# johannes-graeter/limo

Hardware: NVIDIA H100
Metric: BA windows/s (30 KF, 3k LM, 40k obs) (higher is better)
Workload: dtype f64

## Files before the change

limo_b200/csrc/kba_device.cuh:

```cuda
#pragma once
#include <cstdint>
#include <cuda_runtime.h>

namespace kba {

constexpr int kMaxKf = 128;
constexpr int kMaxCam = 8;
constexpr int kPoseStride = 12;
constexpr int kCamStride = 16;
constexpr int kIterLogCap = 160;
constexpr int kFusedMaxKf = 32;

struct WinDesc {
    int n_kf, n_cam, n_lm, n_obs, n_gp;
    int kf_off, cam_off, lm_off, obs_off, gp_off;
    int chunk_off, n_chunks;
    int grp_off, n_groups;
    int scale_kf0, scale_kf1;
    double scale_weight, scale_value;
    double plane_reg_weight;
    int plane_dist_fixed, landmarks_fixed;
    int speed_kf, pad0;
    double speed_weight, speed_dt;
    double speed_v_before[3];
// ... 320 lines not shown
#pragma unroll
    for (int i = 0; i < 3; ++i) {
        T m0, m1, m2;
        if (i == 0) { m0 = fz * (cam[0] - xn * cam[6]); m1 = fz * (cam[1] - xn * cam[7]); m2 = fz * (cam[2] - xn * cam[8]); }
        else if (i == 1) { m0 = fz * (cam[3] - yn * cam[6]); m1 = fz * (cam[4] - yn * cam[7]); m2 = fz * (cam[5] - yn * cam[8]); }
        else { m0 = sqd * cam[6]; m1 = sqd * cam[7]; m2 = sqd * cam[8]; }
        if (write_jp) {
            T* o = jp + (size_t)(6 * i) * stride;
            lin_store<T, kCs>(o, T(-2) * (m1 * a2 - m2 * a1));
            lin_store<T, kCs>(o + stride, T(-2) * (m2 * a0 - m0 * a2));
            lin_store<T, kCs>(o + 2 * stride, T(-2) * (m0 * a1 - m1 * a0));
            lin_store<T, kCs>(o + 3 * stride, m0);
            lin_store<T, kCs>(o + 4 * stride, m1);
            lin_store<T, kCs>(o + 5 * stride, m2);
        }
        if (kJl) {
            T* q = jl + (size_t)(3 * i) * stride;
            lin_store<T, kCs>(q, m0 * pose[0] + m1 * pose[3] + m2 * pose[6]);
            lin_store<T, kCs>(q + stride, m0 * pose[1] + m1 * pose[4] + m2 * pose[7]);
            lin_store<T, kCs>(q + 2 * stride, m0 * pose[2] + m1 * pose[5] + m2 * pose[8]);
        }
    }
    return true;
}

__device__ __forceinline__ double lin_load(const double* base, size_t idx, int precision) {
    return precision ? (double)reinterpret_cast<const float*>(base)[idx] : base[idx];
}

__device__ inline void stage_window(const WinDesc& wd, const double* __restrict__ pose7, const double* __restrict__ cam16,
                                    double* s_pose, double* s_cam) {
    for (int k = threadIdx.x; k < wd.n_kf; k += blockDim.x) {
        const double* p = pose7 + 7 * (size_t)(wd.kf_off + k);
        double R[9];
        quat_to_rot<double>(p, R);
#pragma unroll
        for (int i = 0; i < 9; ++i) s_pose[kPoseStride * k + i] = R[i];
        s_pose[kPoseStride * k + 9] = p[4];
        s_pose[kPoseStride * k + 10] = p[5];
        s_pose[kPoseStride * k + 11] = p[6];
    }
    for (int i = threadIdx.x; i < wd.n_cam * kCamStride; i += blockDim.x) s_cam[i] = cam16[(size_t)wd.cam_off * kCamStride + i];
}

__device__ inline void write_rt(double* rt12, const double* p7) {
    quat_to_rot<double>(p7, rt12);
    rt12[9] = p7[4]; rt12[10] = p7[5]; rt12[11] = p7[6];
}

__device__ __forceinline__ size_t vobs_index(size_t obs_off, int p0, int p1, int o, int c) {
    return 18 * (obs_off + (size_t)p0) + (size_t)(6 * (p1 - p0)) * c + (size_t)6 * (o - p0);
}

__device__ __forceinline__ uint32_t smem_u32(const void* p) { return (uint32_t)__cvta_generic_to_shared(p); }
__device__ __forceinline__ void mbar_init(uint64_t* bar, int count) {
    asm volatile("mbarrier.init.shared::cta.b64 [%0], %1;" ::"r"(smem_u32(bar)), "r"(count));
}
__device__ __forceinline__ void mbar_expect_tx(uint64_t* bar, uint32_t bytes) {
    asm volatile("mbarrier.arrive.expect_tx.shared::cta.b64 _, [%0], %1;" ::"r"(smem_u32(bar)), "r"(bytes) : "memory");
}
__device__ __forceinline__ void tma_load_1d(void* dst, const void* src, uint32_t bytes, uint64_t* bar) {
    asm volatile("cp.async.bulk.shared::cluster.global.mbarrier::complete_tx::bytes [%0], [%1], %2, [%3];" ::"r"(smem_u32(dst)),
                 "l"(src), "r"(bytes), "r"(smem_u32(bar))
                 : "memory");
}
__device__ __forceinline__ void mbar_wait(uint64_t* bar, uint32_t parity) {
    uint32_t done = 0;
    while (!done)
        asm volatile("{\n.reg .pred p;\nmbarrier.try_wait.parity.shared::cta.b64 p, [%1], %2;\nselp.u32 %0, 1, 0, p;\n}"
                     : "=r"(done)
                     : "r"(smem_u32(bar)), "r"(parity)
                     : "memory");
}

__device__ inline void stage_window_bulk(const WinDesc& wd, const double* __restrict__ rt, const double* __restrict__ cam16,
                                         double* s_pose, double* s_cam, uint64_t* bar) {
    if (threadIdx.x == 0) {
        mbar_init(bar, 1);
        asm volatile("fence.proxy.async.shared::cta;" ::: "memory");
    }
    __syncthreads();
    if (threadIdx.x == 0) {
        const uint32_t bp = (uint32_t)(wd.n_kf * kPoseStride * sizeof(double)), bc = (uint32_t)(wd.n_cam * kCamStride * sizeof(double));
        mbar_expect_tx(bar, bp + bc);
        tma_load_1d(s_pose, rt + (size_t)kPoseStride * wd.kf_off, bp, bar);
        tma_load_1d(s_cam, cam16 + (size_t)kCamStride * wd.cam_off, bc, bar);
    }
    mbar_wait(bar, 0);
}

__device__ inline double warp_sum(double v) {
#pragma unroll
    for (int o = 16; o > 0; o >>= 1) v += __shfl_xor_sync(0xffffffffu, v, o);
    return v;
}
__device__ inline double warp_max(double v) {
#pragma unroll
    for (int o = 16; o > 0; o >>= 1) v = fmax(v, __shfl_xor_sync(0xffffffffu, v, o));
    return v;
}

}
```

limo_b200/csrc/kba_kernels.cu:

```cuda
#include "kba_device.cuh"
#include "kba_kernels.h"
#include "kba_regularisers.cuh"
#include "kba_prep.cuh"
#include "kba_linearize.cuh"

#include <cfloat>
#include <cstdio>
#include <cstdlib>
#include <cmath>
#include <type_traits>

namespace kba {

constexpr int kBeginThreads = 1024;
__global__ void __launch_bounds__(kBeginThreads) k_solve_begin(BatchDev bd, SolveParams sp) {
    const int w = blockIdx.x;
    WinState& st = bd.state[w];
    if (st.phase != PH_SOLVE_BEGIN) return;
    const WinDesc wd = bd.desc[w];
    __shared__ int s_has[kMaxKf];
    __shared__ int s_plane[kMaxKf];
    __shared__ int s_cnt[3];
    __shared__ int s_tile_chunk[513];
    for (int k = threadIdx.x; k < wd.n_kf; k += blockDim.x) { s_has[k] = 0; s_plane[k] = 0; }
// ... 1478 lines not shown
            if (off < 0) continue;
            if (bd.obs_rank[base + o] != 0) continue;
            const double* q = pcol + (off - prow0);
#pragma unroll
            for (int r = 0; r < 6; ++r) {
                const double d = delta_f[off + r];
                t[0] += q[r] * d; t[1] += q[prs + r] * d; t[2] += q[2 * prs + r] * d;
            }
        }
    }
    const unsigned any = __ballot_sync(0xffffffffu, mine) & (0xffffu << (threadIdx.x & 16));
    if (gl >= 0 && hl < 10 && !(any != 0u && hl < 6)) {
        const int row = gp_row(bd, wd, bd.gp_kf[wd.gp_off + gl], hl);
        if (row >= 0) {
            const double d = delta_f[row];
#pragma unroll
            for (int c = 0; c < 3; ++c) t[c] += bd.vgp[(size_t)(3 * hl + c) * bd.tot_gp + wd.gp_off + gl] * d;
        }
    }
#pragma unroll
    for (int c = 0; c < 3; ++c)
#pragma unroll
        for (int m = 8; m >= 1; m >>= 1) t[c] += __shfl_xor_sync(0xffffffffu, t[c], m);
    if (have && hl == 0) {
        if (!in) {
            pn[0] = pc[0]; pn[1] = pc[1]; pn[2] = pc[2];
        } else {
            const double* z = bd.lm_z + 3 * (size_t)L;
            const double* li = bd.lm_linv + 6 * (size_t)L;
            const double t0 = t[0] + z[0], t1 = t[1] + z[1], t2 = t[2] + z[2];
            const double d0 = -(li[0] * t0 + li[1] * t1 + li[3] * t2);
            const double d1 = -(li[2] * t1 + li[4] * t2);
            const double d2 = -(li[5] * t2);
            const double* g = bd.lm_g + 3 * (size_t)L;
            const double* lam = bd.lm_lambda + 3 * (size_t)L;
            pn[0] = pc[0] + d0; pn[1] = pc[1] + d1; pn[2] = pc[2] + d2;
            model = -(g[0] * d0 + g[1] * d1 + g[2] * d2) + lam[0] * d0 * d0 + lam[1] * d1 * d1 + lam[2] * d2 * d2;
            step_sq = d0 * d0 + d1 * d1 + d2 * d2;
            xn_sq = pc[0] * pc[0] + pc[1] * pc[1] + pc[2] * pc[2];
            gmax = fmax(fabs(g[0]), fmax(fabs(g[1]), fabs(g[2])));
            if (!isfinite(d0) || !isfinite(d1) || !isfinite(d2)) model = nan("");
        }
    }
    if (hl == 0) { s_red[grp][0] = model; s_red[grp][1] = step_sq; s_red[grp][2] = xn_sq; s_red[grp][3] = gmax; }
    __syncthreads();
    if (threadIdx.x == 0) {
        double a = 0, b = 0, c = 0, g = 0;
        for (int q = 0; q < 16; ++q) { a += s_red[q][0]; b += s_red[q][1]; c += s_red[q][2]; g = fmax(g, s_red[q][3]); }
        double* out = bd.bs_part + ((size_t)w * bd.bs_parts + blockIdx.x) * 4;
        out[0] = a; out[1] = b; out[2] = c; out[3] = g;
    }
}

template <bool kLoop>
__global__ void __launch_bounds__(256) k_backsub_v(BatchDev bd, int n_units) {
    const int w = blockIdx.y;
    const WinState& st = bd.state[w];
    if (st.phase != PH_ITERATE) return;
    const WinDesc& wd = bd.desc[w];
    __shared__ double s_red[16][4];
    const int hl = threadIdx.x & 15, grp = threadIdx.x >> 4;
    for (int unit = blockIdx.x; unit < n_units; unit += gridDim.x) {
    const int j = unit * 16 + grp;
    double model = 0.0, step_sq = 0.0, xn_sq = 0.0, gmax = 0.0;
    const bool have = j < wd.n_lm;
    const int L = wd.lm_off + (have ? j : 0);
    const double* pc = bd.lm[st.cur] + 3 * (size_t)L;
    double* pn = bd.lm[1 - st.cur] + 3 * (size_t)L;
    const int* lm_ptr = bd.lm_ptr + wd.lm_off + w;
    const int o0 = have ? lm_ptr[j] : 0, o1 = have ? lm_ptr[j + 1] : 0;
    const bool in = have && bd.lm_active[L] && o1 > o0 && !wd.landmarks_fixed && !st.solve_failed;
    const size_t base = (size_t)wd.obs_off;
    const double* delta_f = bd.delta_f + (size_t)w * bd.nr_cap_max;
    double t[3] = {0, 0, 0};
    if (in) {
        for (int o = o0 + hl; o < o1; o += 16) {
            const int off = bd.obs_row[base + o];
            if (off < 0) continue;
            double d[6];
#pragma unroll
            for (int r = 0; r < 6; ++r) d[r] = delta_f[off + r];
#pragma unroll
            for (int c = 0; c < 3; ++c) {
                const double2* v = reinterpret_cast<const double2*>(bd.vobs + vobs_index(base, o0, o1, o, c));
#pragma unroll
                for (int h = 0; h < 3; ++h) {
                    const double2 x = v[h];
                    t[c] += x.x * d[2 * h] + x.y * d[2 * h + 1];
                }
            }
        }
        const int gl = (wd.n_gp > 0) ? bd.gp_of_lm[L] : -1;
        if (gl >= 0 && hl < 10) {
            const int row = gp_row(bd, wd, bd.gp_kf[wd.gp_off + gl], hl);
            if (row >= 0) {
                const double d = delta_f[row];
#pragma unroll
                for (int c = 0; c < 3; ++c) t[c] += bd.vgp[(size_t)(3 * hl + c) * bd.tot_gp + wd.gp_off + gl] * d;
            }
        }
    }
#pragma unroll
    for (int c = 0; c < 3; ++c)
#pragma unroll
        for (int m = 8; m >= 1; m >>= 1) t[c] += __shfl_xor_sync(0xffffffffu, t[c], m);
    if (have && hl == 0) {
        if (!in) {
            pn[0] = pc[0]; pn[1] = pc[1]; pn[2] = pc[2];
        } else {
            const double* z = bd.lm_z + 3 * (size_t)L;
            const double* li = bd.lm_linv + 6 * (size_t)L;
            const double t0 = t[0] + z[0], t1 = t[1] + z[1], t2 = t[2] + z[2];
            const double d0 = -(li[0] * t0 + li[1] * t1 + li[3] * t2);
            const double d1 = -(li[2] * t1 + li[4] * t2);
            const double d2 = -(li[5] * t2);
            const double* g = bd.lm_g + 3 * (size_t)L;
            const double* lam = bd.lm_lambda + 3 * (size_t)L;
            pn[0] = pc[0] + d0; pn[1] = pc[1] + d1; pn[2] = pc[2] + d2;
            model = -(g[0] * d0 + g[1] * d1 + g[2] * d2) + lam[0] * d0 * d0 + lam[1] * d1 * d1 + lam[2] * d2 * d2;
            step_sq = d0 * d0 + d1 * d1 + d2 * d2;
            xn_sq = pc[0] * pc[0] + pc[1] * pc[1] + pc[2] * pc[2];
            gmax = fmax(fabs(g[0]), fmax(fabs(g[1]), fabs(g[2])));
            if (!isfinite(d0) || !isfinite(d1) || !isfinite(d2)) model = nan("");
        }
    }
    if (hl == 0) { s_red[grp][0] = model; s_red[grp][1] = step_sq; s_red[grp][2] = xn_sq; s_red[grp][3] = gmax; }
    __syncthreads();
    if (threadIdx.x == 0) {
        double a = 0, b = 0, c = 0, g = 0;
        for (int q = 0; q < 16; ++q) { a += s_red[q][0]; b += s_red[q][1]; c += s_red[q][2]; g = fmax(g, s_red[q][3]); }
        double* out = bd.bs_part + ((size_t)w * bd.bs_parts + unit) * 4;
        out[0] = a; out[1] = b; out[2] = c; out[3] = g;
    }
    if constexpr (!kLoop) break;
    if (unit + (int)gridDim.x < n_units) __syncthreads();
    }
}

__device__ void log_iter(BatchDev& bd, int w, WinState& st, double cost, double cost_change, double gmax,
                         double step_norm, double rel, double radius, int valid, int successful) {
    if (st.log_n >= kIterLogCap) return;
// ... 513 lines not shown
            k_landmark_reduce<true><<<dim3((bd.max_lm + 15) / 16, B), 256, 0, s>>>(bd, sp); LCHK("k_landmark_reduce");
            k_obs_v2<<<g_obs, 256, 0, s>>>(bd); LCHK("k_obs_v2");
        }
        const dim3 gf(bd.p_split, B);
        if (lc.fused_slots == 7) k_schur_fused<7><<<gf, 512, schur_fused_smem(), s>>>(bd);
        else k_schur_fused<6><<<gf, 512, schur_fused_smem(), s>>>(bd);
        LCHK("k_schur_fused");
    } else {
        k_landmark_reduce<false><<<dim3((bd.max_lm + 15) / 16, B), 256, 0, s>>>(bd, sp); LCHK("k_landmark_reduce");
        for (int round = 0; round <= lc.max_rank; ++round) k_obs_v<<<g_obs, 256, 0, s>>>(bd, round);
        LCHK("k_obs_v");
        if (bd.tot_gp > 0) k_gp_panel<<<dim3((bd.max_gp * 10 + 255) / 256, B), 256, 0, s>>>(bd);
        LCHK("k_gp_panel");
    }
    if (bd.fused) {
    } else if (lc.small_syrk) {
        k_schur_syrk_tma<<<dim3(bd.p_split, B), 512, schur_tma_smem(), s>>>(bd); LCHK("k_schur_syrk_tma");
    } else {
        const int nb = lc.nr_cap_max / 64;
        k_schur_syrk<<<dim3(nb * (nb + 1) / 2, bd.p_split, B), 256, schur_smem(), s>>>(bd); LCHK("k_schur_syrk");
    }
    const dim3 g_red((lc.nr_cap_max * lc.nr_cap_max + 255) / 256, B);
    BatchDev bc = bd;
    if (bd.sharded) {
        if (bd.p_split > 1) k_sred_reduce<<<g_red, 256, 0, s>>>(bd, 1);
        LCHK("k_sred_reduce");
        const LaunchCfg::WinDescHost& wh = lc.shard_win;
        const long long n_s = (long long)wh.nr_cap * wh.nr_cap, n_b = (long long)wh.n_kf * 27, n_x = n_s + n_b + bd.cost_parts + 2;
        k_shard_pack<<<(unsigned)((n_x + 255) / 256), 256, 0, s>>>(bd); LCHK("k_shard_pack");
        if (int rc = lc.xchg.allreduce(lc.xchg.user, bd.x_send, bd.x_recv, n_x, 0, s)) return rc;
        k_shard_flags<<<1, 32, 0, s>>>(bd); LCHK("k_shard_flags");
        bc.sred = bd.x_recv; bc.bkf = bd.x_recv + n_s; bc.cost_part_x = bd.x_recv + n_s + n_b;
        k_sred_reduce<<<g_red, 256, 0, s>>>(bc, 2); LCHK("k_sred_reduce");
    } else if (bd.p_split > 1) {
        k_sred_reduce<<<g_red, 256, 0, s>>>(bd, 0); LCHK("k_sred_reduce");
    }
    if (bd.solve_tiled) {
        k_reduced_solve<true><<<B, 512, solve_tiled_smem(lc.nr_cap_max), s>>>(bc, sp, 0); LCHK("k_reduced_solve");
    } else if (!bd.solve_split) {
        k_reduced_solve<false><<<B, 512, solve_smem(lc.nr_cap_max), s>>>(bc, sp, 0); LCHK("k_reduced_solve");
    } else {
        k_reduced_solve<false><<<B, 512, solve_smem(lc.nr_cap_max), s>>>(bc, sp, 1); LCHK("k_reduced_solve");
        const int strips = (lc.nr_cap_max + 7) / 8;
        for (int kb = 0; kb < lc.nr_cap_max; kb += kNB) {
            k_chol_diag<<<B, 32, 0, s>>>(bc, kb); LCHK("k_chol_diag");
            k_chol_panel<<<dim3((strips + 15) / 16, B), 512, 0, s>>>(bc, kb); LCHK("k_chol_panel");
            k_chol_trail<<<dim3(bd.solve_split, B), 512, trail_smem(lc.nr_cap_max), s>>>(bc, kb); LCHK("k_chol_trail");
        }
        k_reduced_solve<false><<<B, 512, solve_smem(lc.nr_cap_max), s>>>(bc, sp, 2); LCHK("k_reduced_solve");
    }
    if (bd.fused) {
        const int n_units = (bd.max_lm + 15) / 16;
        const int gx = strided_grid(lc.bs_grid, n_units, 1, 3, B, lc.sm_count, 2, 8);
        if (gx < n_units) k_backsub_v<true><<<dim3(gx, B), 256, 0, s>>>(bd, n_units);
        else k_backsub_v<false><<<dim3(n_units, B), 256, 0, s>>>(bd, n_units);
    }
    else k_backsub<<<dim3((bd.max_lm + 15) / 16, B), 256, 0, s>>>(bd);
    LCHK("k_backsub");
    launch_eval_obs<false>(bd, sp, s);
    if (bd.tot_gp > 0) k_gp_eval<false><<<B, 256, 0, s>>>(bd, sp);
    LCHK("k_gp_eval");
    if (bd.sharded) {
        k_shard_scalars<<<1, 256, 0, s>>>(bd); LCHK("k_shard_scalars");
        if (int rc = lc.xchg.allreduce(lc.xchg.user, bd.xs, bd.xs, 16 + bd.shard_world, 0, s)) return rc;
    }
    k_lm_update<<<(B * 32 + 127) / 128, 128, 0, s>>>(bd, sp); LCHK("k_lm_update");
    k_trim_eval<<<g_lm, 256, 0, s>>>(bd, sp); LCHK("k_trim_eval");
    if (bd.sharded) {
        k_shard_trim_scatter<<<(bd.max_lm + 255) / 256, 256, 0, s>>>(bd); LCHK("k_shard_trim_scatter");
        if (int rc = lc.xchg.allreduce(lc.xchg.user, bd.trim_send, bd.trim_glob, 3LL * bd.lm_total, 0, s)) return rc;
    }
    k_trim_select<<<B, 512, 0, s>>>(bd, sp); LCHK("k_trim_select");
    if (cnt) {
        const int gp = bd.tot_gp > 0 ? 1 : 0;
        const int prep = lin1 ? 1 : 2 + (bd.fused ? 1 : lc.max_rank + 1 + gp);
        const int split = (!bd.solve_tiled && bd.solve_split) ? 1 + 3 * ((lc.nr_cap_max + kNB - 1) / kNB) : 0;
        cnt->launches_total += (bd.fused ? 0 : 1) + 1 + 1 + gp + prep + 1 + (bd.p_split > 1 ? 1 : 0) + 1 + split + 1 + 1 + gp + 1 + 2;
        cnt->launches_jacobian += 1; cnt->launches_prep += prep + gp; cnt->launches_schur += 1; cnt->launches_solve += 2;
        cnt->launches_backsub += 1; cnt->launches_cost += 1 + gp; cnt->launches_update += 1; cnt->launches_trim += 2;
    }
    return 0;
}

void launch_count_active(const BatchDev& bd, cudaStream_t s) {
    cudaMemsetAsync(bd.n_active, 0, sizeof(int), s);
    k_count_active<<<(bd.n_win + 127) / 128, 128, 0, s>>>(bd); LCHK("k_count_active");
}

__global__ void __launch_bounds__(256) k_loop_cond(BatchDev bd, cudaGraphConditionalHandle handle, int* pass, int max_passes) {
    int active = 0;
    for (int w = threadIdx.x; w < bd.n_win; w += blockDim.x) active += (bd.state[w].phase != PH_DONE) ? 1 : 0;
    active = __syncthreads_count(active > 0);
    if (threadIdx.x == 0) {
        const int p = *pass + 1;
        *pass = p;
        *bd.n_active = active;
        cudaGraphSetConditional(handle, (active > 0 && p < max_passes) ? 1u : 0u);
    }
}
void launch_loop_cond(const BatchDev& bd, unsigned long long handle, int* pass, int max_passes, cudaStream_t s) {
    k_loop_cond<<<1, 256, 0, s>>>(bd, (cudaGraphConditionalHandle)handle, pass, max_passes);
}

__global__ void k_force_linearize(BatchDev bd) {
    const int w = blockIdx.x * blockDim.x + threadIdx.x;
    if (w >= bd.n_win) return;
    WinState& st = bd.state[w];
    st.phase = PH_ITERATE; st.need_linearize = 1; st.iter0 = 1; st.cur = 0; st.eval_failed = 0; st.solve_failed = 0;
// ... 31 lines not shown
```

limo_b200/csrc/kba_linearize.cuh:

```cuda
#pragma once
#include <type_traits>
#include "kba_device.cuh"

namespace kba {

constexpr int kLinThreads = 256;
constexpr int kLinWarps = kLinThreads / 32;

__host__ __device__ __forceinline__ int lin_tile_bound(int n_obs, int n_lm) { return n_obs / 16 + n_lm / 32 + 4; }
__device__ __forceinline__ size_t lin_tile_offset(const WinDesc& wd, int w) {
    return (size_t)(wd.obs_off / 16) + (size_t)(wd.lm_off / 32) + 4 * (size_t)w;
}

__device__ inline void build_lin_tiles(const BatchDev& bd, const WinDesc& wd, WinState& st, int w, int* s_chunk ) {
    const int* lm_ptr = bd.lm_ptr + wd.lm_off + w;
    int2* tiles = bd.lin_tile + lin_tile_offset(wd, w);
    const int per = max(64, (wd.n_lm + 511) / 512);
    const int n_chunks = (wd.n_lm + per - 1) / per;
    for (int pass = 0; pass < 2; ++pass) {
        for (int c = threadIdx.x; c < n_chunks; c += blockDim.x) {
            const int j0 = c * per, j1 = min(wd.n_lm, j0 + per);
            int n = 0, t_start = 0, t_cnt = 0;
            int2* out = tiles + (pass ? s_chunk[c] : 0);
            int o0 = lm_ptr[j0];
// ... 173 lines not shown
#pragma unroll
            for (int e = 0; e < 3; ++e) {
                tt[e] = st.iter0 ? 1.0 + sqrt(cd[e]) : tt_ld[e];
                const double t2 = tt[e] * tt[e];
                lam[e] = fmin(fmax(cd[e], sp.min_lm_diagonal * t2), sp.max_lm_diagonal * t2) * inv_radius;
            }
            const double a00 = c[0] + lam[0], a11 = c[3] + lam[1], a22 = c[5] + lam[2];
            const double i00 = rsqrt(a00);
            const double l10 = c[1] * i00, l20 = c[2] * i00;
            const double d11 = a11 - l10 * l10;
            const double i11 = rsqrt(d11);
            const double l21 = (c[4] - l20 * l10) * i11;
            const double d22 = a22 - l20 * l20 - l21 * l21;
            const double i22 = rsqrt(d22);
            if (!((a00 > 0.0) && (d11 > 0.0) && (d22 > 0.0))) {
                st.solve_failed = 1;
            } else {
                const double i10 = -l10 * i00 * i11;
                const double i21 = -l21 * i11 * i22;
                const double i20 = -(l20 * i00 + l21 * i10) * i22;
                if (first) {
                    double* li = bd.lm_linv + 6 * (size_t)L;
                    li[0] = i00; li[1] = i10; li[2] = i11; li[3] = i20; li[4] = i21; li[5] = i22;
                    double* zz = bd.lm_z + 3 * (size_t)L;
                    zz[0] = i00 * g[0]; zz[1] = i10 * g[0] + i11 * g[1]; zz[2] = i20 * g[0] + i21 * g[1] + i22 * g[2];
#pragma unroll
                    for (int e = 0; e < 3; ++e) {
                        bd.lm_g[3 * (size_t)L + e] = g[e];
                        bd.lm_lambda[3 * (size_t)L + e] = lam[e];
                        if (st.iter0) bd.lm_scale[3 * (size_t)L + e] = tt[e];
                    }
                    if (gl >= 0) {
                        for (int rr = 0; rr < 10; ++rr) {
                            const double jf_ = bd.gp_lin[(1 + rr) * TG + G];
                            const double e0 = jf_ * gjl[0], e1 = jf_ * gjl[1], e2 = jf_ * gjl[2];
                            bd.vgp[(3 * rr + 0) * TG + G] = e0 * i00;
                            bd.vgp[(3 * rr + 1) * TG + G] = e0 * i10 + e1 * i11;
                            bd.vgp[(3 * rr + 2) * TG + G] = e0 * i20 + e1 * i21 + e2 * i22;
                        }
                    }
                }
                if ((six[5][lane] & 128) && six[1][lane] >= 0) {
                    const double* R = s_pose + kPoseStride * six[0][lane];
                    const int g0 = six[2][lane];
                    double wm[9];
#pragma unroll
                    for (int r = 0; r < 3; ++r) {
                        const double m0 = sma[sym3(r, 0)], m1 = sma[sym3(r, 1)], m2 = sma[sym3(r, 2)];
                        const double l0 = m0 * R[0] + m1 * R[3] + m2 * R[6], l1 = m0 * R[1] + m1 * R[4] + m2 * R[7], l2 = m0 * R[2] + m1 * R[5] + m2 * R[8];
                        wm[3 * r + 0] = l0 * i00;
                        wm[3 * r + 1] = l0 * i10 + l1 * i11;
                        wm[3 * r + 2] = l0 * i20 + l1 * i21 + l2 * i22;
                    }
#pragma unroll
                    for (int cc = 0; cc < 3; ++cc) {
                        double2* out = reinterpret_cast<double2*>(bd.vobs + vobs_index(0, g0, g0 + klen, g0 + lane - seg0, cc));
                        const double w0 = wm[cc], w1 = wm[3 + cc], w2 = wm[6 + cc];
                        const double a0 = sma[6], a1 = sma[7], a2 = sma[8];
                        out[0] = make_double2(2.0 * (a1 * w2 - a2 * w1), 2.0 * (a2 * w0 - a0 * w2));
                        out[1] = make_double2(2.0 * (a0 * w1 - a1 * w0), w0);
                        out[2] = make_double2(w1, w2);
                    }
                }
            }
        }
    }
    __syncthreads();
    if (tid == 0) {
        double s = 0.0;
        int cnt = 0;
        for (int q = 0; q < kLinWarps; ++q) { s += s_red[q]; cnt += s_cnt[q]; }
        if (want_cost()) bd.cost_part_x[(size_t)w * bd.cost_parts + unit] = s;
        if (cnt) atomicAdd(bd.jac_obs, (unsigned long long)cnt);
    }
    if constexpr (!kLoop) break;
    if (unit + (int)gridDim.x < n_units) __syncthreads();
    }
}

}
```

limo_b200/csrc/kba_schur_fused.cuh:

```cuda
#pragma once

namespace kba {

constexpr int kLG = 8;
constexpr int kGC = 3 * kLG;
constexpr int kFStages = 6;
constexpr int kFMaxRs = 196;
constexpr int kFStageDoubles = kGC * kFMaxRs;
constexpr int kFObs = 128;
constexpr int kFConsumerWarps = 12;
constexpr int kFMaxKf = 32;

__constant__ signed char kSyrkMap12[12][7] = {
    {72, 7, 22, 33, 36, 48, 65}, {67, 10, 12, 19, 40, 53, -1}, {73, 1, 13, 17, 42, 50, -1}, {77, 8, 21, 26, 39, 54, -1},
    {75, 3, 18, 34, 49, 57, -1}, {69, 6, 23, 41, 58, 62, -1},  {66, 11, 27, 32, 38, 64, -1}, {74, 9, 20, 30, 37, 52, 55},
    {68, 0, 14, 16, 31, 44, 51}, {76, 2, 24, 29, 43, 45, 60},  {71, 5, 25, 28, 46, 56, 63},  {70, 4, 15, 35, 47, 59, 61}};

__device__ __forceinline__ void mbar_arrive(uint64_t* bar) {
    asm volatile("mbarrier.arrive.shared::cta.b64 _, [%0];" ::"r"(smem_u32(bar)) : "memory");
}
__device__ __forceinline__ void cp_async_elem(double* dst, const double* src) {
    asm volatile("cp.async.ca.shared.global [%0], [%1], 8;" ::"r"(smem_u32(dst)), "l"(src) : "memory");
}
__device__ __forceinline__ void cp_async_elem(float* dst, const float* src) {
    asm volatile("cp.async.ca.shared.global [%0], [%1], 4;" ::"r"(smem_u32(dst)), "l"(src) : "memory");
}
__device__ __forceinline__ void cp_async16(double* dst, const double* src) {
    asm volatile("cp.async.cg.shared.global [%0], [%1], 16;" ::"r"(smem_u32(dst)), "l"(src) : "memory");
}
__device__ __forceinline__ void cp_async8(double* dst, const double* src) {
    asm volatile("cp.async.ca.shared.global [%0], [%1], 8;" ::"r"(smem_u32(dst)), "l"(src) : "memory");
}
__device__ __forceinline__ void cp_async_arrive(uint64_t* bar) {
    asm volatile("cp.async.mbarrier.arrive.noinc.shared::cta.b64 [%0];" ::"r"(smem_u32(bar)) : "memory");
}
__device__ __forceinline__ void cp_async_commit() { asm volatile("cp.async.commit_group;" ::: "memory"); }
template <int N>
__device__ __forceinline__ void cp_async_wait() { asm volatile("cp.async.wait_group %0;" ::"n"(N) : "memory"); }
__device__ __forceinline__ void producer_sync() { asm volatile("bar.sync 1, 128;" ::: "memory"); }
template <int N>
__device__ __forceinline__ void reg_dec() { asm volatile("setmaxnreg.dec.sync.aligned.u32 %0;" ::"n"(N)); }
template <int N>
__device__ __forceinline__ void reg_inc() { asm volatile("setmaxnreg.inc.sync.aligned.u32 %0;" ::"n"(N)); }

constexpr size_t schur_fused_smem() { return (size_t)kFStages * kFStageDoubles * sizeof(double) + 24 * sizeof(uint64_t); }

#ifdef KBA_PROF
#define KBA_PROF_DECL long long pt_ = clock64(), pacc_[3] = {0, 0, 0}
#define KBA_PROF_T0 pt_ = clock64()
#define KBA_PROF_ACC(i) do { const long long n_ = clock64(); pacc_[i] += n_ - pt_; pt_ = n_; } while (0)
#define KBA_PROF_FLUSH(base) do { if (lane == 0 && bd.prof) for (int i_ = 0; i_ < 3; ++i_) atomicAdd(bd.prof + (base) + i_, (unsigned long long)pacc_[i_]); } while (0)
#else
#define KBA_PROF_DECL
#define KBA_PROF_T0
#define KBA_PROF_ACC(i)
#define KBA_PROF_FLUSH(base)
#endif

__device__ __forceinline__ void schur_split(int n_groups, int p_split, int& per, int& used) {
    per = max(8, (n_groups + p_split - 1) / p_split);
    used = max(1, min(p_split, (n_groups + per - 1) / per));
}

template <int kSlots>
__global__ void __launch_bounds__(512, 1) k_schur_fused(BatchDev bd) {
    const int w = blockIdx.y;
    const WinState& st = bd.state[w];
    if (st.phase != PH_ITERATE || st.solve_failed) return;
    const WinDesc& wd = bd.desc[w];
    if (wd.landmarks_fixed) return;
    extern __shared__ __align__(128) unsigned char fsm[];
    double* stage = reinterpret_cast<double*>(fsm);
    uint64_t* full = reinterpret_cast<uint64_t*>(fsm + (size_t)kFStages * kFStageDoubles * sizeof(double));
    uint64_t* empty = full + kFStages;
    const int tid = threadIdx.x, warp = tid >> 5, lane = tid & 31;
    const int n_f = st.n_f, nt = (n_f + 8) >> 3, trhs = n_f >> 3;
    int per, used;
    schur_split(wd.n_groups, (int)gridDim.x, per, used);
    if ((int)blockIdx.x >= used) return;
    const int g0 = blockIdx.x * per, g1 = min(wd.n_groups, g0 + per);
    const int* grs = bd.grp_rs + wd.grp_off;
    const int* gt0 = bd.grp_t0 + wd.grp_off;
    const int* gt1 = bd.grp_t1 + wd.grp_off;
    if (tid == 0) {
        for (int i = 0; i < kFStages; ++i) { mbar_init(&full[i], 1); mbar_init(&empty[i], kFConsumerWarps); }
        asm volatile("fence.proxy.async.shared::cta;" ::: "memory");
    }
    __syncthreads();
    auto next_group = [&](int g) { while (g < g1 && grs[g] == 0) ++g; return g; };

    if (warp >= kFConsumerWarps) {
        if (kSlots == 7) reg_dec<56>(); else reg_dec<104>();

        const int pw = warp - kFConsumerWarps;
        const int* lm_ptr = bd.lm_ptr + wd.lm_off + w;
        const size_t base = (size_t)wd.obs_off, TG = (size_t)bd.tot_gp;
        const bool sync_path = wd.n_gp > 0 || wd.max_rank > 0;
        const int cj = lane / 3, cc = lane - 3 * cj;
        const int zj = lane - 24;
        int g1_ = -1, rs1 = 0, t01 = 0, t11 = 0, act1 = 0, p01 = 0, p11 = 0;
        int4 run1 = make_int4(0, 0, 0, 0);
        KBA_PROF_DECL;
        auto load_meta = [&](int g) {
            g1_ = g; act1 = 0; run1 = make_int4(0, 0, 0, 0); p01 = p11 = 0;
            if (g >= g1) return;
            rs1 = grs[g]; t01 = gt0[g]; t11 = gt1[g];
            if (lane < 24) {
                const int j = g * kLG + cj;
                if (j < wd.n_lm) { run1 = bd.lm_run[wd.lm_off + j]; p01 = lm_ptr[j]; p11 = lm_ptr[j + 1]; }
            } else {
                const int j = g * kLG + zj;
                if (j < wd.n_lm) { act1 = bd.lm_active[wd.lm_off + j]; p01 = lm_ptr[j]; p11 = lm_ptr[j + 1]; }
            }
        };
        auto nth_group = [&](int g, int n) {
            g = next_group(g);
            for (; n > 0 && g < g1; --n) g = next_group(g + 1);
            return g;
        };
        int g = nth_group(g0, pw), gi = pw;
        load_meta(g);
        while (g < g1) {
            const int rs = rs1, t0 = t01, t1 = t11, act0 = act1, p00 = p01, p10 = p11;
            const int4 run0 = run1;
            const int gnext = nth_group(g + 1, 3);
            load_meta(gnext);
            const int slot = gi % kFStages;
            KBA_PROF_T0;
            if (gi >= kFStages) mbar_wait(&empty[slot], ((gi / kFStages) - 1) & 1);
            KBA_PROF_ACC(0);
            double* sb = stage + (size_t)slot * kFStageDoubles;
            {
                const int h = rs >> 1;
                for (int c = 0; c < kGC; ++c)
                    for (int r2 = lane; r2 < h; r2 += 32) reinterpret_cast<double2*>(sb + (size_t)c * kFMaxRs)[r2] = make_double2(0.0, 0.0);
            }
            const bool no_run = lane < 24 && (run0.y < 0 || (run0.y > 0 && ((run0.z - 8 * t0) & 1)));
            const bool bulk = __ballot_sync(0xffffffffu, no_run) == 0u && !sync_path;
            asm volatile("fence.proxy.async.shared::cta;" ::: "memory");
            __syncwarp();
            KBA_PROF_ACC(1);
            const int j0 = g * kLG, j1 = min(wd.n_lm, j0 + kLG);
            const int ob = lm_ptr[j0], oe = lm_ptr[j1];
            const int rl = (trhs >= t0 && trhs < t1) ? n_f - 8 * t0 : 8 * (t1 - t0) + (n_f - 8 * trhs);
            if (bulk) {
                if (lane < 24 && run0.y > 0) {
                    const uint32_t bytes = (uint32_t)(48 * run0.y);
                    asm volatile("mbarrier.expect_tx.relaxed.cta.shared::cta.b64 [%0], %1;" ::"r"(smem_u32(&full[slot])), "r"(bytes) : "memory");
                    tma_load_1d(sb + (size_t)(3 * cj + cc) * kFMaxRs + (run0.z - 8 * t0),
                                bd.vobs + vobs_index(base, p00, p10, p00 + run0.x, cc), bytes, &full[slot]);
                }
            } else {
                for (int o = ob + lane; o < oe; o += 32) {
                    const size_t oo = base + o;
                    const int row = bd.obs_row[oo];
                    if (row < 0 || bd.obs_rank[oo] != 0) continue;
                    const int lm = bd.obs_lm[oo], q0 = lm_ptr[lm], q1 = lm_ptr[lm + 1];
                    double* dst = sb + (size_t)(3 * (lm - j0)) * kFMaxRs + (row - 8 * t0);
#pragma unroll
                    for (int c = 0; c < 3; ++c) {
                        const double* src = bd.vobs + vobs_index(base, q0, q1, o, c);
                        if (((row - 8 * t0) & 1) == 0) {
#pragma unroll
                            for (int h = 0; h < 3; ++h) cp_async16(dst + c * kFMaxRs + 2 * h, src + 2 * h);
                        } else {
#pragma unroll
                            for (int r = 0; r < 6; ++r) cp_async8(dst + c * kFMaxRs + r, src + r);
                        }
                    }
                }
            }
            if (lane >= 24 && act0 && p10 > p00) {
                const double* zz = bd.lm_z + 3 * (size_t)(wd.lm_off + j0 + zj);
                double* col = sb + (size_t)(3 * zj) * kFMaxRs + rl;
                cp_async8(col, zz); cp_async8(col + kFMaxRs, zz + 1); cp_async8(col + 2 * kFMaxRs, zz + 2);
            }
            if (!sync_path) {
                asm volatile("cp.async.mbarrier.arrive.shared::cta.b64 [%0];" ::"r"(smem_u32(&full[slot])) : "memory");
                __syncwarp();
                if (lane == 0) mbar_arrive(&full[slot]);
            } else {
                cp_async_commit();
                cp_async_wait<0>();
                __syncwarp();
                for (int round = 1; round <= wd.max_rank; ++round) {
                    for (int o = ob + lane; o < oe; o += 32) {
                        const size_t oo = base + o;
                        const int row = bd.obs_row[oo];
                        if (row < 0 || bd.obs_rank[oo] != round) continue;
                        const int lm = bd.obs_lm[oo], q0 = lm_ptr[lm], q1 = lm_ptr[lm + 1];
                        double* dst = sb + (size_t)(3 * (lm - j0)) * kFMaxRs + (row - 8 * t0);
                        for (int c = 0; c < 3; ++c) {
                            const double* src = bd.vobs + vobs_index(base, q0, q1, o, c);
                            for (int r = 0; r < 6; ++r) dst[c * kFMaxRs + r] += src[r];
                        }
                    }
                    __syncwarp();
                }
                if (wd.n_gp > 0) {
                    for (int it = lane; it < 80; it += 32) {
                        const int jj = it / 10, r = it - 10 * jj, j = j0 + jj;
                        const int L = wd.lm_off + j;
                        if (j >= wd.n_lm || !bd.lm_active[L] || lm_ptr[j + 1] <= lm_ptr[j]) continue;
// ... 60 lines not shown
#pragma unroll
            for (int s = 0; s < kSlots; ++s) {
                const int bi = my_bi[s], bj = my_bj[s];
                if (bj < b0 || bj >= b1) continue;
                if (bi >= b0 && bi < b1) {
                    const double* pa = sb + 16 * (bi - b0);
                    const double* pb = sb + 16 * (bj - b0);
                    if (bi != bj) {
#pragma unroll
                        for (int kk = 0; kk < kGC; kk += 4) {
                            const double a0 = pa[kk * kFMaxRs], a1 = pa[kk * kFMaxRs + 8], b0v = pb[kk * kFMaxRs], b1v = pb[kk * kFMaxRs + 8];
                            dmma(acc[s][0][0], acc[s][0][1], a0, b0v);
                            dmma(acc[s][1][0], acc[s][1][1], a0, b1v);
                            dmma(acc[s][2][0], acc[s][2][1], a1, b0v);
                            dmma(acc[s][3][0], acc[s][3][1], a1, b1v);
                        }
                    } else {
#pragma unroll
                        for (int kk = 0; kk < kGC; kk += 4) {
                            const double a0 = pa[kk * kFMaxRs], a1 = pa[kk * kFMaxRs + 8];
                            dmma(acc[s][0][0], acc[s][0][1], a0, a0);
                            dmma(acc[s][2][0], acc[s][2][1], a1, a0);
                            dmma(acc[s][3][0], acc[s][3][1], a1, a1);
                        }
                    }
                } else if (bi == brhs && !rhs_in) {
                    const double* pa = sb + rhs_row;
                    const double* pb = sb + 16 * (bj - b0);
                    if (trhs & 1) {
#pragma unroll
                        for (int kk = 0; kk < kGC; kk += 4) {
                            const double a1 = pa[kk * kFMaxRs], b0v = pb[kk * kFMaxRs], b1v = pb[kk * kFMaxRs + 8];
                            dmma(acc[s][2][0], acc[s][2][1], a1, b0v);
                            dmma(acc[s][3][0], acc[s][3][1], a1, b1v);
                        }
                    } else {
#pragma unroll
                        for (int kk = 0; kk < kGC; kk += 4) {
                            const double a0 = pa[kk * kFMaxRs], b0v = pb[kk * kFMaxRs], b1v = pb[kk * kFMaxRs + 8];
                            dmma(acc[s][0][0], acc[s][0][1], a0, b0v);
                            dmma(acc[s][1][0], acc[s][1][1], a0, b1v);
                        }
                    }
                }
            }
            __syncwarp();
            if (lane == 0) mbar_arrive(&empty[slot]);
            KBA_PROF_ACC(1);
            g = gn; t0 = t0n; t1 = t1n;
        }
        KBA_PROF_FLUSH(0);
    }
    double* out = bd.sred + wd.s_off * (size_t)bd.p_split + (size_t)blockIdx.x * wd.nr_cap * wd.nr_cap;
#pragma unroll
    for (int s = 0; s < kSlots; ++s) {
        const int bi = my_bi[s], bj = my_bj[s];
        if (bi >= nb2) continue;
#pragma unroll
        for (int q = 0; q < 4; ++q) {
            const int i = 2 * bi + (q >> 1), j = 2 * bj + (q & 1);
            if (i >= nt || j > i) continue;
            double* o = out + (size_t)(8 * i + fr) * wd.nr_cap + 8 * j + 2 * fc;
            o[0] = acc[s][q][0];
            o[1] = acc[s][q][1];
        }
    }
}

}
```

Before: 1108.

## Store compact W/a per observation and rebuild V columns on the fly

Linearization now writes a compact 12-double record per observation (the 3x3 W matrix plus the a vector) in place of the expanded 18-double V block, and back-substitution and the fused Schur producer rebuild the V columns from it with cross products. This cuts the global memory traffic for vobs at the cost of extra FLOPs and of giving up the TMA bulk-copy path. The producer also issues an L2 prefetch per landmark group and, when the stage is reused, zeroes only the previously written cells instead of clearing the whole stage. Several paths depend on lin1, and the rank/GP sync paths keep the old vobs indexing, so consistency relies on lin1 being set only where the new layout is written.

```diff
diff --git a/limo_b200/csrc/kba_device.cuh b/limo_b200/csrc/kba_device.cuh
--- a/limo_b200/csrc/kba_device.cuh
+++ b/limo_b200/csrc/kba_device.cuh
@@ -396,6 +396,25 @@
     return 18 * (obs_off + (size_t)p0) + (size_t)(6 * (p1 - p0)) * c + (size_t)6 * (o - p0);
 }
 
+__device__ __forceinline__ size_t vobs_wa_index(size_t obs_off, int o) { return 12 * (obs_off + (size_t)o); }
+
+__device__ __forceinline__ void vobs_wa_load(const double* __restrict__ src, double wa[12]) {
+    const double2* s = reinterpret_cast<const double2*>(src);
+#pragma unroll
+    for (int h = 0; h < 6; ++h) {
+        const double2 x = s[h];
+        wa[2 * h] = x.x; wa[2 * h + 1] = x.y;
+    }
+}
+
+__device__ __forceinline__ void v_column(const double w[3], const double a[3], double v[6]) {
+    const double w0 = w[0], w1 = w[1], w2 = w[2], a0 = a[0], a1 = a[1], a2 = a[2];
+    v[0] = 2.0 * __fma_rn(a1, w2, -__dmul_rn(a2, w1));
+    v[1] = 2.0 * __fma_rn(a2, w0, -__dmul_rn(a0, w2));
+    v[2] = 2.0 * __fma_rn(a0, w1, -__dmul_rn(a1, w0));
+    v[3] = w0; v[4] = w1; v[5] = w2;
+}
+
 __device__ __forceinline__ uint32_t smem_u32(const void* p) { return (uint32_t)__cvta_generic_to_shared(p); }
 __device__ __forceinline__ void mbar_init(uint64_t* bar, int count) {
     asm volatile("mbarrier.init.shared::cta.b64 [%0], %1;" ::"r"(smem_u32(bar)), "r"(count));
diff --git a/limo_b200/csrc/kba_kernels.cu b/limo_b200/csrc/kba_kernels.cu
--- a/limo_b200/csrc/kba_kernels.cu
+++ b/limo_b200/csrc/kba_kernels.cu
@@ -1554,7 +1554,7 @@
     }
 }
 
-template <bool kLoop>
+template <bool kLoop, bool kWA>
 __global__ void __launch_bounds__(256) k_backsub_v(BatchDev bd, int n_units) {
     const int w = blockIdx.y;
     const WinState& st = bd.state[w];
@@ -1582,13 +1582,25 @@
             double d[6];
 #pragma unroll
             for (int r = 0; r < 6; ++r) d[r] = delta_f[off + r];
-#pragma unroll
-            for (int c = 0; c < 3; ++c) {
-                const double2* v = reinterpret_cast<const double2*>(bd.vobs + vobs_index(base, o0, o1, o, c));
-#pragma unroll
-                for (int h = 0; h < 3; ++h) {
-                    const double2 x = v[h];
-                    t[c] += x.x * d[2 * h] + x.y * d[2 * h + 1];
+            if constexpr (kWA) {
+                double wa[12];
+                vobs_wa_load(bd.vobs + vobs_wa_index(base, o), wa);
+#pragma unroll
+                for (int c = 0; c < 3; ++c) {
+                    double v[6];
+                    v_column(wa + 3 * c, wa + 9, v);
+#pragma unroll
+                    for (int h = 0; h < 3; ++h) t[c] += __fma_rn(v[2 * h], d[2 * h], __dmul_rn(v[2 * h + 1], d[2 * h + 1]));
+                }
+            } else {
+#pragma unroll
+                for (int c = 0; c < 3; ++c) {
+                    const double2* v = reinterpret_cast<const double2*>(bd.vobs + vobs_index(base, o0, o1, o, c));
+#pragma unroll
+                    for (int h = 0; h < 3; ++h) {
+                        const double2 x = v[h];
+                        t[c] += x.x * d[2 * h] + x.y * d[2 * h + 1];
+                    }
                 }
             }
         }
@@ -2208,8 +2220,13 @@
     if (bd.fused) {
         const int n_units = (bd.max_lm + 15) / 16;
         const int gx = strided_grid(lc.bs_grid, n_units, 1, 3, B, lc.sm_count, 2, 8);
-        if (gx < n_units) k_backsub_v<true><<<dim3(gx, B), 256, 0, s>>>(bd, n_units);
-        else k_backsub_v<false><<<dim3(n_units, B), 256, 0, s>>>(bd, n_units);
+        if (lin1) {
+            if (gx < n_units) k_backsub_v<true, true><<<dim3(gx, B), 256, 0, s>>>(bd, n_units);
+            else k_backsub_v<false, true><<<dim3(n_units, B), 256, 0, s>>>(bd, n_units);
+        } else {
+            if (gx < n_units) k_backsub_v<true, false><<<dim3(gx, B), 256, 0, s>>>(bd, n_units);
+            else k_backsub_v<false, false><<<dim3(n_units, B), 256, 0, s>>>(bd, n_units);
+        }
     }
     else k_backsub<<<dim3((bd.max_lm + 15) / 16, B), 256, 0, s>>>(bd);
     LCHK("k_backsub");
diff --git a/limo_b200/csrc/kba_linearize.cuh b/limo_b200/csrc/kba_linearize.cuh
--- a/limo_b200/csrc/kba_linearize.cuh
+++ b/limo_b200/csrc/kba_linearize.cuh
@@ -249,15 +249,13 @@
                         wm[3 * r + 1] = l0 * i10 + l1 * i11;
                         wm[3 * r + 2] = l0 * i20 + l1 * i21 + l2 * i22;
                     }
-#pragma unroll
-                    for (int cc = 0; cc < 3; ++cc) {
-                        double2* out = reinterpret_cast<double2*>(bd.vobs + vobs_index(0, g0, g0 + klen, g0 + lane - seg0, cc));
-                        const double w0 = wm[cc], w1 = wm[3 + cc], w2 = wm[6 + cc];
-                        const double a0 = sma[6], a1 = sma[7], a2 = sma[8];
-                        out[0] = make_double2(2.0 * (a1 * w2 - a2 * w1), 2.0 * (a2 * w0 - a0 * w2));
-                        out[1] = make_double2(2.0 * (a0 * w1 - a1 * w0), w0);
-                        out[2] = make_double2(w1, w2);
-                    }
+                    double2* out = reinterpret_cast<double2*>(bd.vobs + vobs_wa_index(0, g0 + lane - seg0));
+                    out[0] = make_double2(wm[0], wm[3]);
+                    out[1] = make_double2(wm[6], wm[1]);
+                    out[2] = make_double2(wm[4], wm[7]);
+                    out[3] = make_double2(wm[2], wm[5]);
+                    out[4] = make_double2(wm[8], sma[6]);
+                    out[5] = make_double2(sma[7], sma[8]);
                 }
             }
         }
diff --git a/limo_b200/csrc/kba_schur_fused.cuh b/limo_b200/csrc/kba_schur_fused.cuh
--- a/limo_b200/csrc/kba_schur_fused.cuh
+++ b/limo_b200/csrc/kba_schur_fused.cuh
@@ -33,6 +33,9 @@
 }
 __device__ __forceinline__ void cp_async_arrive(uint64_t* bar) {
     asm volatile("cp.async.mbarrier.arrive.noinc.shared::cta.b64 [%0];" ::"r"(smem_u32(bar)) : "memory");
+}
+__device__ __forceinline__ void prefetch_l2(const void* src, uint32_t bytes) {
+    asm volatile("cp.async.bulk.prefetch.L2.global [%0], %1;" ::"l"(src), "r"(bytes) : "memory");
 }
 __device__ __forceinline__ void cp_async_commit() { asm volatile("cp.async.commit_group;" ::: "memory"); }
 template <int N>
@@ -73,6 +76,7 @@
     double* stage = reinterpret_cast<double*>(fsm);
     uint64_t* full = reinterpret_cast<uint64_t*>(fsm + (size_t)kFStages * kFStageDoubles * sizeof(double));
     uint64_t* empty = full + kFStages;
+    int* slot_grp = reinterpret_cast<int*>(empty + kFStages);
     const int tid = threadIdx.x, warp = tid >> 5, lane = tid & 31;
     const int n_f = st.n_f, nt = (n_f + 8) >> 3, trhs = n_f >> 3;
     int per, used;
@@ -83,7 +87,7 @@
     const int* gt0 = bd.grp_t0 + wd.grp_off;
     const int* gt1 = bd.grp_t1 + wd.grp_off;
     if (tid == 0) {
-        for (int i = 0; i < kFStages; ++i) { mbar_init(&full[i], 1); mbar_init(&empty[i], kFConsumerWarps); }
+        for (int i = 0; i < kFStages; ++i) { mbar_init(&full[i], 1); mbar_init(&empty[i], kFConsumerWarps); slot_grp[i] = -1; }
         asm volatile("fence.proxy.async.shared::cta;" ::: "memory");
     }
     __syncthreads();
@@ -98,6 +102,24 @@
         const bool sync_path = wd.n_gp > 0 || wd.max_rank > 0;
         const int cj = lane / 3, cc = lane - 3 * cj;
         const int zj = lane - 24;
+        const bool keep_zero = kSlots != 7 && bd.lin1 && !sync_path;
+        if (keep_zero) {
+            for (int i = tid - 32 * kFConsumerWarps; i < kFStages * kFStageDoubles / 2; i += 128)
+                reinterpret_cast<double2*>(stage)[i] = make_double2(0.0, 0.0);
+            producer_sync();
+        }
+        const auto rhs_row = [&](int t0, int t1) {
+            return (trhs >= t0 && trhs < t1) ? n_f - 8 * t0 : 8 * (t1 - t0) + (n_f - 8 * trhs);
+        };
+        const auto zero_block = [&](double* dst, bool even) {
+            if (even) {
+#pragma unroll
+                for (int h = 0; h < 3; ++h) reinterpret_cast<double2*>(dst)[h] = make_double2(0.0, 0.0);
+            } else {
+#pragma unroll
+                for (int r = 0; r < 6; ++r) dst[r] = 0.0;
+            }
+        };
         int g1_ = -1, rs1 = 0, t01 = 0, t11 = 0, act1 = 0, p01 = 0, p11 = 0;
         int4 run1 = make_int4(0, 0, 0, 0);
         KBA_PROF_DECL;
@@ -126,29 +148,95 @@
             const int gnext = nth_group(g + 1, 3);
             load_meta(gnext);
             const int slot = gi % kFStages;
+            if (bd.lin1 && lane == 0) {
+                const int q0 = lm_ptr[g * kLG], q1 = lm_ptr[min(wd.n_lm, g * kLG + kLG)];
+                if (q1 > q0) prefetch_l2(bd.vobs + vobs_wa_index(base, q0), (uint32_t)(96 * (q1 - q0)));
+            }
             KBA_PROF_T0;
             if (gi >= kFStages) mbar_wait(&empty[slot], ((gi / kFStages) - 1) & 1);
             KBA_PROF_ACC(0);
             double* sb = stage + (size_t)slot * kFStageDoubles;
-            {
+            if (keep_zero) {
+                const int gp = slot_grp[slot];
+                if (gp >= 0) {
+                    const int pj0 = gp * kLG, pt0 = gt0[gp];
+                    const int qb = lm_ptr[pj0], qe = lm_ptr[min(wd.n_lm, pj0 + kLG)];
+                    for (int o = qb + lane; o < qe; o += 32) {
+                        const int row = bd.obs_row[base + o], lm = bd.obs_lm[base + o];
+                        if (row < 0) continue;
+                        double* dst = sb + (size_t)(3 * (lm - pj0)) * kFMaxRs + (row - 8 * pt0);
+                        const bool even = ((row - 8 * pt0) & 1) == 0;
+#pragma unroll
+                        for (int c = 0; c < 3; ++c) zero_block(dst + c * kFMaxRs, even);
+                    }
+                    if (lane < kGC) sb[(size_t)lane * kFMaxRs + rhs_row(pt0, gt1[gp])] = 0.0;
+                }
+                if (lane == 0) slot_grp[slot] = g;
+            } else {
                 const int h = rs >> 1;
                 for (int c = 0; c < kGC; ++c)
                     for (int r2 = lane; r2 < h; r2 += 32) reinterpret_cast<double2*>(sb + (size_t)c * kFMaxRs)[r2] = make_double2(0.0, 0.0);
             }
             const bool no_run = lane < 24 && (run0.y < 0 || (run0.y > 0 && ((run0.z - 8 * t0) & 1)));
-            const bool bulk = __ballot_sync(0xffffffffu, no_run) == 0u && !sync_path;
+            const bool bulk = !bd.lin1 && __ballot_sync(0xffffffffu, no_run) == 0u && !sync_path;
             asm volatile("fence.proxy.async.shared::cta;" ::: "memory");
             __syncwarp();
             KBA_PROF_ACC(1);
             const int j0 = g * kLG, j1 = min(wd.n_lm, j0 + kLG);
             const int ob = lm_ptr[j0], oe = lm_ptr[j1];
-            const int rl = (trhs >= t0 && trhs < t1) ? n_f - 8 * t0 : 8 * (t1 - t0) + (n_f - 8 * trhs);
+            const int rl = rhs_row(t0, t1);
             if (bulk) {
                 if (lane < 24 && run0.y > 0) {
                     const uint32_t bytes = (uint32_t)(48 * run0.y);
                     asm volatile("mbarrier.expect_tx.relaxed.cta.shared::cta.b64 [%0], %1;" ::"r"(smem_u32(&full[slot])), "r"(bytes) : "memory");
                     tma_load_1d(sb + (size_t)(3 * cj + cc) * kFMaxRs + (run0.z - 8 * t0),
                                 bd.vobs + vobs_index(base, p00, p10, p00 + run0.x, cc), bytes, &full[slot]);
+                }
+            } else if (bd.lin1) {
+                const auto put = [&](double* dst, bool even, const double w[3], const double a[3]) {
+                    double v[6];
+                    v_column(w, a, v);
+                    if (even) {
+#pragma unroll
+                        for (int h = 0; h < 3; ++h) reinterpret_cast<double2*>(dst)[h] = make_double2(v[2 * h], v[2 * h + 1]);
+                    } else {
+#pragma unroll
+                        for (int r = 0; r < 6; ++r) dst[r] = v[r];
+                    }
+                };
+                if constexpr (kSlots == 7) {
+                    for (int o = ob + lane; o < oe; o += 32) {
+                        const int row = bd.obs_row[base + o], lm = bd.obs_lm[base + o];
+                        if (row < 0) continue;
+                        const double* src = bd.vobs + vobs_wa_index(base, o);
+                        double* dst = sb + (size_t)(3 * (lm - j0)) * kFMaxRs + (row - 8 * t0);
+                        const double a[3] = {src[9], src[10], src[11]};
+#pragma unroll 1
+                        for (int c = 0; c < 3; ++c) {
+                            const double w[3] = {src[3 * c], src[3 * c + 1], src[3 * c + 2]};
+                            put(dst + c * kFMaxRs, ((row - 8 * t0) & 1) == 0, w, a);
+                        }
+                    }
+                } else {
+                    for (int o = ob + lane; o < oe; o += 64) {
+                        double wa[2][12];
+                        int row[2], lm[2];
+#pragma unroll
+                        for (int u = 0; u < 2; ++u) {
+                            row[u] = -1; lm[u] = 0;
+                            if (o + 32 * u < oe) {
+                                vobs_wa_load(bd.vobs + vobs_wa_index(base, o + 32 * u), wa[u]);
+                                row[u] = bd.obs_row[base + o + 32 * u]; lm[u] = bd.obs_lm[base + o + 32 * u];
+                            }
+                        }
+#pragma unroll
+                        for (int u = 0; u < 2; ++u) {
+                            if (row[u] < 0) continue;
+                            double* dst = sb + (size_t)(3 * (lm[u] - j0)) * kFMaxRs + (row[u] - 8 * t0);
+#pragma unroll
+                            for (int c = 0; c < 3; ++c) put(dst + c * kFMaxRs, ((row[u] - 8 * t0) & 1) == 0, wa[u] + 3 * c, wa[u] + 9);
+                        }
+                    }
                 }
             } else {
                 for (int o = ob + lane; o < oe; o += 32) {
@@ -315,6 +403,7 @@
         KBA_PROF_FLUSH(0);
     }
     double* out = bd.sred + wd.s_off * (size_t)bd.p_split + (size_t)blockIdx.x * wd.nr_cap * wd.nr_cap;
+    const int nt_out = (reinterpret_cast<const volatile WinState&>(st).n_f + 8) >> 3;
 #pragma unroll
     for (int s = 0; s < kSlots; ++s) {
         const int bi = my_bi[s], bj = my_bj[s];
@@ -322,7 +411,7 @@
 #pragma unroll
         for (int q = 0; q < 4; ++q) {
             const int i = 2 * bi + (q >> 1), j = 2 * bj + (q & 1);
-            if (i >= nt || j > i) continue;
+            if (i >= nt_out || j > i) continue;
             double* o = out + (size_t)(8 * i + fr) * wd.nr_cap + 8 * j + 2 * fc;
             o[0] = acc[s][q][0];
             o[1] = acc[s][q][1];
```

Measured after the change: 1151 (median of 6 runs). 1.04x the previous value.
